# Layr-Labs/rust-kzg-bn254

Measured on AMD Instinct MI355X. Metric: G1-MSM (scalar,point) pairs/s = 2^20 x KZG coeff-form commitments/s, 2^20-point SRS, higher is better.
Workload: dtype int32x9 (29-bit limbs, 64-bit accumulate); 1 GPU; G1 MSM 2^20 scalars (KZG::commit_coeff_form), scalars resident in HBM; step k commits buffer k mod 8 (8 distinct resident scalar sets, 256 MiB); pipeline_depth=2, steps_per_launch=1

## Files before the change

rust-kzg-bn254_amd/csrc/curve_quad.h:

```cpp
#pragma once
#include "curve_pair.h"

#if defined(__HIPCC__)
namespace kzg {

struct QuadXyzz {
    Fq c;
    bool inf;
};

__device__ __forceinline__ void quad_set_inf(QuadXyzz& h) { fe_set_zero(h.c); h.inf = true; }

constexpr int QUAD_BCAST0 = 0x00, QUAD_BCAST1 = 0x55, QUAD_BCAST2 = 0xAA, QUAD_BCAST3 = 0xFF, QUAD_SWAP2 = 0x4E ;
template <int CTRL>
__device__ __forceinline__ int32_t quad_mov(int32_t x) {
#ifdef KZG_QUAD_NO_DPP
    const int lane = (int)(threadIdx.x & 63u);
    return __shfl(x, (lane & ~3) | ((CTRL >> (2 * (lane & 3))) & 3), 64);
#else
    return __builtin_amdgcn_mov_dpp(x, CTRL, 0xF, 0xF, true);
#endif
}
template <int CTRL>
__device__ __forceinline__ void fe_quad_mov(Fq& r, const Fq& a) {
// ... 93 lines not shown
    quad_add_tail(r, acc.c, df, sq, !acc.inf, from, q);
    if (acc.inf) r = from;
}

__device__ __forceinline__ void quad_dbl(QuadXyzz& r, const QuadXyzz& a, uint32_t q) {
    Fq y, u, s1, t1;
    fe_quad_mov<QUAD_BCAST1>(y, a.c);
    fe_dbl(u, y); fe_norm(u);
    fe_select(s1, q == 0u, a.c, u);
    fe_sqr(t1, s1);
    Fq m, m0, v1;
    fe_add(m, t1, t1); fe_add(m, m, t1); fe_norm(m);
    fe_quad_mov<QUAD_BCAST0>(m0, m);
    fe_quad_mov<QUAD_BCAST1>(v1, t1);
    Fq a2, b2, t2;
    fe_select(a2, q == 1u, u, a.c);
    fe_select(a2, q == 3u, m0, a2);
    fe_select(b2, q == 3u, m0, v1);
    fe_mul(t2, a2, b2);
    Fq mm, w1, x3, tq;
    fe_quad_mov<QUAD_BCAST3>(mm, t2);
    fe_quad_mov<QUAD_BCAST1>(w1, t2);
    fe_sub(x3, mm, t2); fe_sub(x3, x3, t2); fe_norm(x3);
    fe_add(tq, t2, t2); fe_add(tq, tq, t2); fe_sub(tq, tq, mm); fe_norm(tq);
    Fq a3, b3, t3;
    fe_select(a3, q == 0u, m, w1);
    fe_select(b3, q == 0u, tq, a.c);
    fe_mul(t3, a3, b3);
    Fq d0, y3;
    fe_quad_mov<QUAD_BCAST0>(d0, t3);
    fe_sub(y3, d0, t3); fe_norm(y3);
    Fq lo, hi;
    fe_select(lo, q == 1u, y3, x3);
    fe_select(hi, q == 3u, t3, t2);
    fe_select(r.c, q >= 2u, hi, lo);
    r.inf = false;
}
__device__ __forceinline__ void quad_dbl_any(QuadXyzz& r, const QuadXyzz& a, uint32_t q) {
    if (__all(a.inf)) { r = a; return; }
    QuadXyzz d;
    quad_dbl(d, a, q);
    if (a.inf) r = a; else r = d;
}

__device__ __forceinline__ void quad_load(QuadXyzz& h, const int32_t* __restrict__ base, size_t stride, size_t i, uint32_t q) {
#pragma unroll
    for (int j = 0; j < NL; ++j) h.c.l[j] = base[(size_t)(q * NL + j) * stride + i];
    const int z = fe_is_literal_zero(h.c) ? 1 : 0;
    h.inf = quad_mov<QUAD_BCAST2>(z) != 0;
}
__device__ __forceinline__ void quad_store(int32_t* __restrict__ base, size_t stride, size_t i, const QuadXyzz& h, uint32_t q) {
#pragma unroll
    for (int j = 0; j < NL; ++j) base[(size_t)(q * NL + j) * stride + i] = h.inf ? 0 : h.c.l[j];
}
__device__ __forceinline__ void quad_store_wire(uint32_t* __restrict__ out_wire, size_t i, const QuadXyzz& h, uint32_t q) {
    uint32_t w[8];
    if (h.inf) {
#pragma unroll
        for (int j = 0; j < 8; ++j) w[j] = 0;
    } else {
        fe_to_wire(w, h.c);
    }
    uint32_t* p = out_wire + i * 32 + q * 8;
    *reinterpret_cast<uint4*>(p) = make_uint4(w[0], w[1], w[2], w[3]);
    *reinterpret_cast<uint4*>(p + 4) = make_uint4(w[4], w[5], w[6], w[7]);
}
__device__ __forceinline__ void quad_shfl_down(QuadXyzz& r, const QuadXyzz& h, int d) {
#pragma unroll
    for (int j = 0; j < NL; ++j) r.c.l[j] = __shfl_down(h.c.l[j], d, 64);
    r.inf = __shfl_down((int)h.inf, d, 64) != 0;
}
__device__ __forceinline__ void quad_shfl(QuadXyzz& r, const QuadXyzz& h, int src) {
#pragma unroll
    for (int j = 0; j < NL; ++j) r.c.l[j] = __shfl(h.c.l[j], src, 64);
    r.inf = __shfl((int)h.inf, src, 64) != 0;
}

#ifndef KZG_PAIR_WAVES
#define KZG_PAIR_WAVES 3
#endif
#ifndef KZG_QUAD_SMALL_WAVES
#define KZG_QUAD_SMALL_WAVES 4
#endif
__device__ void group_zeta64(HalfXyzz& v, uint32_t lane, uint32_t w, bool odd, int32_t* __restrict__ lds);
__device__ void group_zeta64q(QuadXyzz& v, uint32_t lane, uint32_t w, uint32_t q, int32_t* __restrict__ lds);
struct PairLanes {
    using Point = HalfXyzz;
    using Role = bool;
    static constexpr uint32_t LANES = 2, GROUPS = 64 / LANES, LOG_GROUPS = 5;
    static constexpr int THREADS = 128, WAVES = KZG_PAIR_WAVES;
    static constexpr int ZETA_LDS_WORDS = 2 * NL * 64;
    static constexpr uint32_t FUSED_HEAVY = 12;
    static __device__ __forceinline__ Role role(uint32_t lane) { return (lane & 1u) != 0; }
    static __device__ __forceinline__ int affine_half(Role r) { return r ? 2 : 0; }
    static __device__ __forceinline__ void set_inf(Point& h) { half_set_inf(h); }
    static __device__ __forceinline__ void load(Point& h, const int32_t* __restrict__ base, size_t stride, size_t i, Role r) { half_load(h, base, stride, i, r); }
    static __device__ __forceinline__ void store(int32_t* __restrict__ base, size_t stride, size_t i, const Point& h, Role r) { half_store(base, stride, i, h, r); }
    static __device__ __forceinline__ void store_wire(uint32_t* __restrict__ out_wire, size_t i, const Point& h, Role r) { half_store_wire(out_wire, i, h, r); }
    static __device__ __forceinline__ void add(Point& r, const Point& a, const Point& b, Role role) { pair_add(r, a, b, role); }
    static __device__ __forceinline__ void madd(Point& r, const Point& acc, const Fq& c, uint32_t neg, Role role) { pair_madd(r, acc, c, neg, role); }
    static __device__ __forceinline__ void shfl_down(Point& r, const Point& h, int d) { half_shfl_down(r, h, d); }
    static __device__ __forceinline__ void shfl(Point& r, const Point& h, int src) { half_shfl(r, h, src); }
    static constexpr auto& zeta64 = group_zeta64;
};
struct QuadLanes {
    using Point = QuadXyzz;
    using Role = uint32_t;
    static constexpr uint32_t LANES = 4, GROUPS = 64 / LANES, LOG_GROUPS = 4;
    static constexpr int THREADS = 256, WAVES = KZG_QUAD_SMALL_WAVES;
    static constexpr int ZETA_LDS_WORDS = (NL + 1) * 256;
    static constexpr uint32_t FUSED_HEAVY = 8;
    static __device__ __forceinline__ Role role(uint32_t lane) { return lane & 3u; }
    static __device__ __forceinline__ int affine_half(Role r) { return (r & 1u) ? 2 : 0; }
    static __device__ __forceinline__ void set_inf(Point& h) { quad_set_inf(h); }
    static __device__ __forceinline__ void load(Point& h, const int32_t* __restrict__ base, size_t stride, size_t i, Role r) { quad_load(h, base, stride, i, r); }
    static __device__ __forceinline__ void store(int32_t* __restrict__ base, size_t stride, size_t i, const Point& h, Role r) { quad_store(base, stride, i, h, r); }
    static __device__ __forceinline__ void store_wire(uint32_t* __restrict__ out_wire, size_t i, const Point& h, Role r) { quad_store_wire(out_wire, i, h, r); }
    static __device__ __forceinline__ void add(Point& r, const Point& a, const Point& b, Role role) { quad_add(r, a, b, role); }
    static __device__ __forceinline__ void madd(Point& r, const Point& acc, const Fq& c, uint32_t neg, Role role) { quad_madd(r, acc, c, neg, role); }
    static __device__ __forceinline__ void shfl_down(Point& r, const Point& h, int d) { quad_shfl_down(r, h, d); }
    static __device__ __forceinline__ void shfl(Point& r, const Point& h, int src) { quad_shfl(r, h, src); }
    static constexpr auto& zeta64 = group_zeta64q;
};

}
#endif
```

rust-kzg-bn254_amd/csrc/msm.hip:

```cpp
#include "engine.h"
#include <new>
#include "msm_kernels.h"
#include "host_msm_epilogue.h"
#include "host_pairing.h"

#include <algorithm>
#include <cstdlib>
#include <chrono>
#include <cstdio>
#include <cstring>
#include <type_traits>
#include <vector>

namespace kzg {

void MsmWorkspace::release() {
    DeviceBuffer* all[] = {&scalars, &bases, &bases_wire, &digits, &sorted, &count, &blockbase, &sort_tmp, &sort_key, &sort_small, &offs, &block_sums,
                           &head, &cont, &blob, &bucket, &chunkS, &chunkTmp, &chunkA, &out_wire};
    for (auto* b : all) b->release();
    if (pinned_out) { (void)hipHostFree(pinned_out); pinned_out = nullptr; }
    if (ev_ready) { for (auto& e : ev) (void)hipEventDestroy(e); ev_ready = false; }
    if (ev_done) { (void)hipEventDestroy(ev_done); ev_done = nullptr; }
    if (ev_sorted) { (void)hipEventDestroy(ev_sorted); ev_sorted = nullptr; }
}
// ... 129 lines not shown
    hipStream_t st = L.st;
    const uint32_t n_total = p.n * p.batch;
    KZG_HIP_TRY(L.ctx, hipMemsetAsync(ws.count.p, 0, (size_t)p.G * 4, st));
    hipLaunchKernelGGL(k_msm_digits, dim3((n_total + 255) / 256), dim3(256), 0, st, L.d_scalars, n_total, p.n, p.c, p.W, ws.digits.as<uint32_t>(), (uint32_t*)nullptr);
    KZG_MARK(1);
    if (p.sort_small) {
        const uint32_t entries = (uint32_t)p.entries(), ge = (uint32_t)((p.entries() + 255) / 256);
        KZG_HIP_TRY(L.ctx, hipMemsetAsync(ws.blockbase.p, 0, (size_t)p.G * 4, st));
        hipLaunchKernelGGL(k_sort_small_hist, dim3(ge), dim3(256), 0, st, ws.digits.as<uint32_t>(), entries, p.set_len, p.B, ws.count.as<uint32_t>());
        scan_counts(L);
        KZG_MARK(2);
        hipLaunchKernelGGL(k_sort_small_scatter, dim3(ge), dim3(256), 0, st, ws.digits.as<uint32_t>(), entries, p.n, p.set_len, p.B,
                           ws.offs.as<uint32_t>(), ws.blockbase.as<uint32_t>(), p.idx_stride, (uint32_t)p.W, ws.sorted.as<uint32_t>());
    } else {
        const size_t lds_bytes = (size_t)p.B * 4;
        hipLaunchKernelGGL(k_sort_hist, dim3(p.tiles), dim3(256), lds_bytes, st, ws.digits.as<uint32_t>(), p.set_len, p.tile_len,
                           p.tiles_per_set, p.B, ws.count.as<uint32_t>(), ws.blockbase.as<uint32_t>());
        scan_counts(L);
        KZG_MARK(2);
        hipLaunchKernelGGL(k_sort_scatter, dim3(p.tiles), dim3(256), lds_bytes, st, ws.digits.as<uint32_t>(), p.n, p.set_len, p.tile_len,
                           p.tiles_per_set, p.B, ws.offs.as<uint32_t>(), ws.blockbase.as<uint32_t>(), p.idx_stride,
                           (uint32_t)p.W, ws.sorted.as<uint32_t>());
    }
    KZG_MARK(3);
    return KZG_OK;
}

static int32_t enqueue_sort(const Launch& L, const PolyPtrs* poly_ptrs) {
    const Plan& p = L.p;
    kzg_ctx* ctx = L.ctx;
    MsmWorkspace& ws = L.ws;
    if (p.bitsum) {
        for (int i = 0; i <= 4; ++i) KZG_MARK(i);
        return KZG_OK;
    }
    { int32_t rc = set_sort_lds_attributes(ctx); if (rc != KZG_OK) return rc; }
    const bool stagger = p.tables && p.polys >= 2;
    if (stagger && ctx->last_sorted && ctx->last_sorted_stream != L.st) KZG_HIP_TRY(ctx, hipStreamWaitEvent(L.st, ctx->last_sorted, 0));
    KZG_MARK(0);
    const uint32_t clean_g = ws.count_zero_ptr == ws.count.p ? ws.count_zero_g : 0;
    ws.count_zero_g = 0;
    const int32_t rc = p.sort2 ? sort_two_level(L, poly_ptrs) : p.lean_sort ? sort_lean(L, clean_g) : sort_from_digits(L);
    if (rc != KZG_OK) return rc;
    KZG_MARK(4);
    if (p.tables) {
        if (!ws.ev_sorted) KZG_HIP_TRY(ctx, hipEventCreateWithFlags(&ws.ev_sorted, hipEventDisableTiming));
        KZG_HIP_TRY(ctx, hipEventRecord(ws.ev_sorted, L.st));
        ctx->last_sorted = ws.ev_sorted;
        ctx->last_sorted_stream = L.st;
    }
    return KZG_OK;
}

static int32_t enqueue_accumulate(const Launch& L) {
    const Plan& p = L.p;
    MsmWorkspace& ws = L.ws;
    if (!p.bitsum && !p.fused)
        dispatch<true, false>(!L.bases.identity_free, [&](auto identity_bases) {
            hipLaunchKernelGGL(k_msm_accumulate<decltype(identity_bases)::value>, dim3(p.nl / 256), dim3(256), 0, L.st, L.bases.points, ws.sorted.as<uint32_t>(),
                               ws.offs.as<uint32_t>(), p.G, ws.head.as<int32_t>(), (size_t)p.G, ws.cont.as<int32_t>(), (size_t)p.nl, p.idx_log, p.stride_adj);
        });
    KZG_MARK(5);
    return KZG_OK;
}

static int32_t reduce_bitsum(const Launch& L) {
    const Plan& p = L.p;
    dispatch<8, 16, 32>(p.bitsum_chunk, [&](auto chunk) {
        hipLaunchKernelGGL(k_bitsum_level1<decltype(chunk)::value>, dim3(p.bitsum_wg), dim3(256), 0, L.st, L.bases.points, L.bases.table_stride, L.d_scalars, p.n,
                           L.ws.chunkS.as<int32_t>());
    });
    KZG_MARK(6);
    hipLaunchKernelGGL(k_bitsum_level2, dim3(p.n_out), dim3(256), 0, L.st, L.ws.chunkS.as<int32_t>(), p.bitsum_wg, L.d_out);
    return KZG_OK;
}

static int32_t reduce_tables(const Launch& L) {
    const Plan& p = L.p;
    MsmWorkspace& ws = L.ws;
    const uint32_t G1 = p.G1(), G1p = p.G1p();
    int32_t* x1 = ws.chunkS.as<int32_t>();
    dispatch<true, false>(p.quad1, [&](auto quads) {
        using LG = std::conditional_t<decltype(quads)::value, QuadLanes, PairLanes>;
        if (p.fused)
            hipLaunchKernelGGL(k_msm_bucket_bits1_fused<LG>, dim3(G1), dim3(LG::THREADS), 0, L.st, L.bases.points, ws.sorted.as<uint32_t>(), ws.offs.as<uint32_t>(), p.B,
                               p.idx_log, p.stride_adj, G1, x1, (size_t)7 * G1, L.d_out);
        else
            hipLaunchKernelGGL(k_msm_bucket_bits1<LG>, dim3(G1), dim3(LG::THREADS), 0, L.st, ws.offs.as<uint32_t>(), p.B, p.nl, ws.head.as<int32_t>(), (size_t)p.G,
                               ws.cont.as<int32_t>(), (size_t)p.nl, G1, x1, (size_t)7 * G1, L.d_out);
    });
    KZG_MARK(6);
    if (p.polys && p.c == 7) {
        hipLaunchKernelGGL(k_batch_finish, dim3((p.polys + 63) / 64), dim3(64), 0, L.st, x1, (size_t)7 * G1, G1, L.d_out);
    } else if (G1 > 1) {
        const uint32_t waves2 = 7 * G1p;
        if (p.quad)
            hipLaunchKernelGGL(k_red_bits2q, dim3(waves2), dim3(256), 0, L.st, x1, (size_t)7 * G1, G1, G1p, L.d_out);
        else
            hipLaunchKernelGGL(k_red_bits2p, dim3((waves2 + 1) / 2), dim3(128), 0, L.st, x1, (size_t)7 * G1, G1, G1p, L.d_out);
    }
    return KZG_OK;
}

static int32_t reduce_generic(const Launch& L) {
    const Plan& p = L.p;
    MsmWorkspace& ws = L.ws;
    hipStream_t st = L.st;
    const uint32_t n_chunks = p.n_chunks(), n_windows = p.n_windows();
    const uint32_t gg = (p.G + 255) / 256;
    hipLaunchKernelGGL(k_msm_bucket_fin, dim3(gg), dim3(256), 0, st, ws.offs.as<uint32_t>(), p.G, p.nl, p.m, n_chunks, ws.head.as<int32_t>(), (size_t)p.G,
                       ws.cont.as<int32_t>(), (size_t)p.nl, ws.bucket.as<int32_t>(), (size_t)p.G);
    const uint32_t gc = (n_chunks + 255) / 256;
    KZG_MARK(6);
    hipLaunchKernelGGL(k_red_chunk_sums, dim3(gc), dim3(256), 0, st, ws.bucket.as<int32_t>(), (size_t)p.G, n_chunks, p.m,
                       ws.chunkS.as<int32_t>(), (size_t)n_chunks);
    hipLaunchKernelGGL(k_red_suffix_scan, dim3(n_windows), dim3(p.T), 0, st, ws.chunkS.as<int32_t>(), ws.chunkTmp.as<int32_t>(),
                       (size_t)n_chunks, p.T);
    hipLaunchKernelGGL(k_red_chunk_running, dim3(gc), dim3(256), 0, st, ws.bucket.as<int32_t>(), (size_t)p.G,
                       ws.chunkS.as<int32_t>(), (size_t)n_chunks, n_chunks, p.T, p.m, ws.chunkA.as<int32_t>());
    hipLaunchKernelGGL(k_red_window_sum, dim3(n_windows), dim3(p.T), 0, st, ws.chunkA.as<int32_t>(), (size_t)n_chunks, p.T,
                       L.d_out);
    return KZG_OK;
}

static int32_t enqueue_reduce(const Launch& L) {
    const int32_t rc = L.p.bitsum ? reduce_bitsum(L) : L.p.tables ? reduce_tables(L) : reduce_generic(L);
    if (rc != KZG_OK) return rc;
    KZG_MARK(7);
    return KZG_OK;
}
#undef KZG_MARK

static PlanContext plan_context(const kzg_ctx* ctx) {
    PlanContext pc;
    pc.msm_c_override = ctx->msm_c_override;
    pc.msm_seg_override = ctx->msm_seg_override;
    pc.reduction_lanes = ctx->reduction_lanes;
    pc.acc_wave_slots = ctx->acc_wave_slots;
    for (int sl = 0; sl < KZG_NUM_SLOTS; ++sl) pc.other_in_flight |= ctx->slot_pending[sl] != nullptr;
    return pc;
}

static DeviceBuffer* ws_buffer(MsmWorkspace& ws, int which) {
    DeviceBuffer* const buffers[WS_BUFFERS] = {&ws.digits, &ws.sorted, &ws.count, &ws.sort_tmp, &ws.sort_key, &ws.sort_small, &ws.blockbase, &ws.offs, &ws.block_sums,
                                               &ws.head, &ws.cont, &ws.bucket, &ws.chunkS, &ws.chunkTmp, &ws.chunkA};
    return buffers[which];
}
int32_t msm_pinned_out(kzg_ctx* ctx, MsmWorkspace& ws) {
    if (ws.pinned_out) return KZG_OK;
    KZG_HIP_TRY(ctx, hipHostMalloc(&ws.pinned_out, (size_t)MSM_MAX_OUT * 32 * 4 + MSM_MAX_PARTS * 4, hipHostMallocDefault));
    KZG_HIP_TRY(ctx, hipHostGetDevicePointer(&ws.pinned_out_dev, ws.pinned_out, 0));
    return KZG_OK;
}
int32_t msm_sort_generic(kzg_ctx* ctx, MsmWorkspace& ws, hipStream_t st, const uint4* d_scalars, const Plan& p) {
    if (p.tables || p.batch != 1 || p.bitsum) return KZG_ERR_INVALID_ARG;
    for (int i : {WS_DIGITS, WS_SORTED, WS_COUNT, WS_BLOCKBASE, WS_OFFS, WS_BLOCK_SUMS}) KZG_HIP_TRY(ctx, ws_buffer(ws, i)->reserve(p.bytes[i]));
    const MsmBases none;
    const Launch L{ctx, ws, st, none, d_scalars, p, nullptr, false};
    const int32_t rc = enqueue_sort(L, nullptr);
    if (rc != KZG_OK) return rc;
    KZG_HIP_TRY(ctx, hipGetLastError());
    return KZG_OK;
}

static int32_t msm_enqueue(kzg_ctx* ctx, MsmWorkspace& ws, hipStream_t st, const MsmBases& bases, const uint4* d_scalars, size_t n,
                           uint32_t batch, Pending* pend, uint32_t out_off = 0, uint32_t out_cap = MSM_MAX_OUT, uint32_t polys = 0,
                           const PolyPtrs* poly_ptrs = nullptr) {
    const Plan p = make_plan(plan_context(ctx), n, bases, batch, polys);
    {
        const char* error = nullptr;
        const int32_t rc = msm_plan_status(p, bases, polys, out_off, out_cap, &error);
// ... 300 lines not shown
```

rust-kzg-bn254_amd/csrc/msm_kernels.h:

```cpp
#pragma once
#include <hip/hip_runtime.h>
#include "curve_pair.h"
#include "curve_quad.h"
#include "naf.h"
#include "msm_limits.h"

namespace kzg {

__device__ __forceinline__ void latency_bound_kernel() {
#if !defined(KZG_NO_SETPRIO)
    __builtin_amdgcn_s_setprio(3);
#endif
}

constexpr uint32_t DIGIT_NONE = 0xFFFFFFFFu;

__global__ void __launch_bounds__(256)
k_msm_digits(const uint4* __restrict__ scalars, uint32_t n_total, uint32_t n, int c, int W, uint32_t* __restrict__ digits,
             uint32_t* __restrict__ count = nullptr ) {
    latency_bound_kernel();
    uint32_t j = blockIdx.x * blockDim.x + threadIdx.x;
    if (j >= n_total) return;
    const uint32_t msm = j / n, i = j - msm * n;
    uint4 lo = scalars[2 * (size_t)j], hi = scalars[2 * (size_t)j + 1];
// ... 902 lines not shown
        xyzz_add(r, acc, v);
        acc = r;
    }
    xyzz_store(chunkS, chunk_stride, t, acc);
}
__global__ void __launch_bounds__(RED_T)
k_red_suffix_scan(int32_t* __restrict__ a, int32_t* __restrict__ b, size_t stride, uint32_t T) {
    uint32_t t = threadIdx.x;
    size_t base = (size_t)blockIdx.x * T;
    int32_t* src = a;
    int32_t* dst = b;
    for (uint32_t d = 1; d < T; d <<= 1) {
        if (t < T) {
            Xyzz v;
            xyzz_load(v, src, stride, base + t);
            if (t + d < T) {
                Xyzz u, r;
                xyzz_load(u, src, stride, base + t + d);
                xyzz_add(r, v, u);
                v = r;
            }
            xyzz_store(dst, stride, base + t, v);
        }
        __syncthreads();
        int32_t* tmp = src; src = dst; dst = tmp;
    }
    if (src != a && t < T) {
        Xyzz v;
        xyzz_load(v, src, stride, base + t);
        xyzz_store(a, stride, base + t, v);
    }
}
__global__ void __launch_bounds__(256)
k_red_chunk_running(const int32_t* __restrict__ bucket, size_t bucket_stride, const int32_t* __restrict__ suffix, size_t chunk_stride,
                    uint32_t n_chunks, uint32_t T, uint32_t m, int32_t* __restrict__ chunkA) {
    uint32_t t = blockIdx.x * blockDim.x + threadIdx.x;
    if (t >= n_chunks) return;
    Xyzz run, acc;
    if ((t % T) + 1 < T) xyzz_load(run, suffix, chunk_stride, t + 1);
    else xyzz_set_inf(run);
    xyzz_set_inf(acc);
    for (uint32_t k = m; k-- > 0;) {
        Xyzz v, r;
        xyzz_load(v, bucket, bucket_stride, (size_t)k * n_chunks + t);
        xyzz_add(r, run, v); run = r;
        xyzz_add(r, acc, run); acc = r;
    }
    xyzz_store(chunkA, chunk_stride, t, acc);
}
__global__ void __launch_bounds__(RED_T)
k_red_window_sum(int32_t* __restrict__ a, size_t stride, uint32_t T, uint32_t* __restrict__ out_wire) {
    uint32_t t = threadIdx.x;
    size_t base = (size_t)blockIdx.x * T;
    for (uint32_t d = T >> 1; d >= 1; d >>= 1) {
        if (t < d) {
            Xyzz v, u, r;
            xyzz_load(v, a, stride, base + t);
            xyzz_load(u, a, stride, base + t + d);
            xyzz_add(r, v, u);
            xyzz_store(a, stride, base + t, r);
        }
        __syncthreads();
    }
    if (t == 0) {
        Xyzz v;
        xyzz_load(v, a, stride, base);
        uint32_t w[32];
        xyzz_to_wire(w, v);
        for (int j = 0; j < 32; ++j) out_wire[(size_t)blockIdx.x * 32 + j] = w[j];
    }
}

__device__ __forceinline__ int zeta_role(uint32_t lane) {
    if (lane == 0) return 6;
    if ((lane & (lane - 1)) != 0) return -1;
    return __ffs((int)lane) - 1;
}
__device__ __forceinline__ void xyzz_store_wire(uint32_t* __restrict__ out_wire, size_t i, const Xyzz& v) {
    uint32_t w[32];
    xyzz_to_wire(w, v);
#pragma unroll
    for (int j = 0; j < 32; j += 4) *reinterpret_cast<uint4*>(out_wire + i * 32 + j) = make_uint4(w[j], w[j + 1], w[j + 2], w[j + 3]);
}
__device__ __forceinline__ void group_zeta64(HalfXyzz& v, uint32_t lane, uint32_t w, bool odd, int32_t* __restrict__ lds ) {
    const uint32_t pair = lane >> 1;
#pragma unroll 1
    for (int k = 0; k < 6; ++k) {
        HalfXyzz u;
        bool on;
        if (k < 5) {
            half_shfl_down(u, v, 2 << k);
            on = ((pair >> k) & 1u) == 0;
        } else {
            if (w == 1) {
#pragma unroll
                for (int j = 0; j < NL; ++j) { lds[j * 64 + lane] = v.inf ? 0 : v.u.l[j]; lds[(NL + j) * 64 + lane] = v.inf ? 0 : v.v.l[j]; }
            }
            __syncthreads();
#pragma unroll
            for (int j = 0; j < NL; ++j) { u.u.l[j] = lds[j * 64 + lane]; u.v.l[j] = lds[(NL + j) * 64 + lane]; }
            u.inf = fe_is_literal_zero(u.v);
            on = w == 0;
        }
        if (on) {
            HalfXyzz r;
            pair_add(r, v, u, odd);
            v = r;
        }
    }
}
__device__ __forceinline__ void group_zeta64q(QuadXyzz& v, uint32_t lane, uint32_t w, uint32_t q, int32_t* __restrict__ lds ) {
    const uint32_t quad = lane >> 2, tid = w * 64 + lane;
#pragma unroll 1
    for (int k = 0; k < 6; ++k) {
        QuadXyzz u;
        bool on;
        if (k < 4) {
            quad_shfl_down(u, v, 4 << k);
            on = ((quad >> k) & 1u) == 0;
        } else {
            const uint32_t bit = 1u << (k - 4);
            if (k == 5) __syncthreads();
            if (w & bit) {
#pragma unroll
                for (int j = 0; j < NL; ++j) lds[j * 256 + tid] = v.c.l[j];
                lds[NL * 256 + tid] = v.inf ? 1 : 0;
            }
            __syncthreads();
            on = (w & bit) == 0;
            const uint32_t src = tid + 64 * bit;
            if (on) {
#pragma unroll
                for (int j = 0; j < NL; ++j) u.c.l[j] = lds[j * 256 + src];
                u.inf = lds[NL * 256 + src] != 0;
            }
        }
        if (on) {
            QuadXyzz r;
            quad_add(r, v, u, q);
            v = r;
        }
    }
}

template <class LG>
__device__ __forceinline__ void bucket_partial_lanes(typename LG::Point& v, const BucketSpan& s, uint32_t k, const int32_t* __restrict__ head, size_t head_stride,
                                                     const int32_t* __restrict__ cont, size_t cont_stride, typename LG::Role role) {
    if (k == 0) { LG::load(v, head, head_stride, s.g, role); return; }
    LG::load(v, cont, cont_stride, bucket_cont_lane(s, k), role);
}
template <class LG>
__device__ __noinline__ void bucket_sum_heavy(typename LG::Point& tot, uint32_t g, uint32_t t1, uint32_t np, uint32_t long_run, uint32_t lane,
                                              const int32_t* __restrict__ head, size_t head_stride, const int32_t* __restrict__ cont, size_t cont_stride) {
    const uint32_t grp = lane / LG::LANES;
    const typename LG::Role role = LG::role(lane);
    BucketSpan h;
    h.g = g; h.t1 = t1; h.np = np; h.long_run = long_run != 0;
    typename LG::Point part;
    LG::set_inf(part);
    const uint32_t loads = (np + LG::GROUPS - 1) / LG::GROUPS;
#pragma unroll 1
    for (uint32_t step = 0; step < loads + LG::LOG_GROUPS; ++step) {
        typename LG::Point u;
        bool on;
        if (step < loads) {
            const uint32_t k = grp + LG::GROUPS * step;
            on = k < np;
            if (on) bucket_partial_lanes<LG>(u, h, k, head, head_stride, cont, cont_stride, role);
        } else {
            const uint32_t d = (LG::GROUPS / 2) >> (step - loads);
            LG::shfl_down(u, part, (int)(LG::LANES * d));
            on = grp < d;
        }
        if (on) {
            typename LG::Point r;
            LG::add(r, part, u, role);
            part = r;
        }
    }
    LG::shfl(tot, part, (int)(lane & (LG::LANES - 1)));
}
template <class LG>
__device__ __forceinline__ void bucket_sum_lanes(typename LG::Point& acc, const BucketSpan& s, uint32_t lane, typename LG::Role role, const int32_t* __restrict__ head,
                                                 size_t head_stride, const int32_t* __restrict__ cont, size_t cont_stride) {
    LG::set_inf(acc);
    const bool heavy = s.np > NP_SERIAL;
    if (!heavy) {
#pragma unroll 1
        for (uint32_t k = 0; k < s.np; ++k) {
            typename LG::Point v, r;
            bucket_partial_lanes<LG>(v, s, k, head, head_stride, cont, cont_stride, role);
            LG::add(r, acc, v, role);
            acc = r;
        }
    }
    unsigned long long todo = __ballot(heavy && (lane & (LG::LANES - 1)) == 0);
    while (todo) {
        const int src = __ffsll((long long)todo) - 1;
        todo &= todo - 1;
        typename LG::Point tot;
        bucket_sum_heavy<LG>(tot, __shfl(s.g, src, 64), __shfl(s.t1, src, 64), __shfl(s.np, src, 64), (uint32_t)__shfl((int)s.long_run, src, 64), lane,
                             head, head_stride, cont, cont_stride);
        if ((int)(lane & ~(LG::LANES - 1)) == src) acc = tot;
    }
}
template <class LG>
__global__ void __launch_bounds__(LG::THREADS) __attribute__((amdgpu_waves_per_eu(LG::WAVES, LG::WAVES)))
k_msm_bucket_bits1(const uint32_t* __restrict__ offs, uint32_t B, uint32_t nl, const int32_t* __restrict__ head, size_t head_stride,
                   const int32_t* __restrict__ cont, size_t cont_stride, uint32_t G1, int32_t* __restrict__ x1, size_t x_stride,
                   uint32_t* __restrict__ out_wire ) {
    latency_bound_kernel();
    __shared__ int32_t lds[LG::ZETA_LDS_WORDS];
    const uint32_t g = blockIdx.x, w = threadIdx.x >> 6, lane = threadIdx.x & 63, gp = w * LG::GROUPS + lane / LG::LANES;
    const typename LG::Role role = LG::role(lane);
    const uint32_t L = acc_seg_len(offs[B], nl);
    const uint32_t bkt = g * 64 + gp;
    BucketSpan s;
    s.g = bkt; s.t1 = 0; s.np = 0; s.long_run = false;
    if (bkt < B && L) s = bucket_span(offs, bkt, L);
    typename LG::Point v;
    bucket_sum_lanes<LG>(v, s, lane, role, head, head_stride, cont, cont_stride);
    LG::zeta64(v, lane, w, role, lds);
    const int zr = zeta_role(gp);
    if (zr < 0) return;
    if (G1 == 1) LG::store_wire(out_wire, (size_t)zr, v, role);
    else LG::store(x1, x_stride, (size_t)zr * G1 + g, v, role);
}
template <class LG>
__device__ __noinline__ void fused_heavy_bucket(typename LG::Point& tot, uint32_t hb, uint32_t he, uint32_t lane, const uint4* __restrict__ points,
                                                const uint32_t* __restrict__ sorted, uint32_t idx_log, uint32_t stride_adj) {
    const uint32_t grp = lane / LG::LANES;
    const typename LG::Role role = LG::role(lane);
    typename LG::Point part;
    LG::set_inf(part);
#pragma unroll 1
    for (uint32_t e = hb + grp; e < he; e += LG::GROUPS) {
        const uint32_t cur = sorted[e];
        const uint4* src = points + 4 * acc_point_index(cur & 0x7FFFFFFFu, idx_log, stride_adj) + LG::affine_half(role);
        const uint4 q0 = src[0], q1 = src[1];
        const uint32_t w32[8] = {q0.x, q0.y, q0.z, q0.w, q1.x, q1.y, q1.z, q1.w};
        int any = (q0.x | q0.y | q0.z | q0.w | q1.x | q1.y | q1.z | q1.w) != 0 ? 1 : 0;
        any |= pair_swap(any);
        if (!any) continue;
        Fq c;
        fe_unpack(c, w32);
        typename LG::Point r;
        LG::madd(r, part, c, cur >> 31, role);
        part = r;
    }
#pragma unroll 1
    for (int d = LG::GROUPS / 2; d >= 1; d >>= 1) {
        typename LG::Point u;
        LG::shfl_down(u, part, (int)LG::LANES * d);
        if (grp < (uint32_t)d) {
            typename LG::Point r;
            LG::add(r, part, u, role);
            part = r;
        }
    }
    LG::shfl(tot, part, (int)(lane & (LG::LANES - 1)));
}
template <class LG>
__global__ void __launch_bounds__(LG::THREADS) __attribute__((amdgpu_waves_per_eu(LG::WAVES, LG::WAVES)))
k_msm_bucket_bits1_fused(const uint4* __restrict__ points, const uint32_t* __restrict__ sorted, const uint32_t* __restrict__ offs, uint32_t B,
                         uint32_t idx_log, uint32_t stride_adj, uint32_t G1, int32_t* __restrict__ x1, size_t x_stride,
                         uint32_t* __restrict__ out_wire ) {
    latency_bound_kernel();
    __shared__ int32_t lds[LG::ZETA_LDS_WORDS];
    const uint32_t g = blockIdx.x, w = threadIdx.x >> 6, lane = threadIdx.x & 63, gp = w * LG::GROUPS + lane / LG::LANES;
    const typename LG::Role role = LG::role(lane);
    const uint32_t bkt = gp * G1 + g;
    uint32_t e = 0, end = 0;
    if (bkt < B) { e = offs[bkt]; end = offs[bkt + 1]; }
    const uint32_t hb = e, he = end;
    const bool heavy = end - e > LG::FUSED_HEAVY;
    if (heavy) end = e;
    typename LG::Point v;
    LG::set_inf(v);
    const uint32_t half = LG::affine_half(role);
    const uint32_t last = end ? end - 1 : 0;
    uint32_t ent = e < end ? sorted[e] : 0u;
    uint32_t ent1 = e < end ? sorted[e + 1 < end ? e + 1 : last] : 0u;
    const uint4* src = points + 4 * acc_point_index(ent & 0x7FFFFFFFu, idx_log, stride_adj) + half;
    uint4 q0 = make_uint4(0, 0, 0, 0), q1 = q0;
    if (e < end) { q0 = src[0]; q1 = src[1]; }
#pragma unroll 1
    for (; e < end; ++e) {
        const uint32_t cur = ent;
        const uint32_t w32[8] = {q0.x, q0.y, q0.z, q0.w, q1.x, q1.y, q1.z, q1.w};
        int any = (q0.x | q0.y | q0.z | q0.w | q1.x | q1.y | q1.z | q1.w) != 0 ? 1 : 0;
        ent = ent1;
        src = points + 4 * acc_point_index(ent & 0x7FFFFFFFu, idx_log, stride_adj) + half;
        q0 = src[0]; q1 = src[1];
        ent1 = sorted[e + 2 < end ? e + 2 : last];
        any |= pair_swap(any);
        if (!any) continue;
        Fq c;
        fe_unpack(c, w32);
        typename LG::Point r;
        LG::madd(r, v, c, cur >> 31, role);
        v = r;
    }
    unsigned long long todo = __ballot(heavy && (lane & (LG::LANES - 1)) == 0);
    while (todo) {
        const int src_lane = __ffsll((long long)todo) - 1;
        todo &= todo - 1;
        typename LG::Point tot;
        fused_heavy_bucket<LG>(tot, __shfl(hb, src_lane, 64), __shfl(he, src_lane, 64), lane, points, sorted, idx_log, stride_adj);
        if ((int)(lane & ~(LG::LANES - 1)) == src_lane) v = tot;
    }
    LG::zeta64(v, lane, w, role, lds);
    const int zr = zeta_role(gp);
    if (zr < 0) return;
    if (G1 == 1) LG::store_wire(out_wire, (size_t)zr, v, role);
    else LG::store(x1, x_stride, (size_t)zr * G1 + g, v, role);
}

__device__ __forceinline__ void group_zeta64_dual(HalfXyzz& vA, HalfXyzz& vB, uint32_t lane, uint32_t w, bool odd, int32_t* __restrict__ lds ) {
    const uint32_t gp = w * 32 + (lane >> 1);
#pragma unroll 1
    for (int k = 0; k < 6; ++k) {
        const bool bit = ((gp >> k) & 1u) != 0;
        HalfXyzz mine, pub, u, r;
        half_select(mine, bit, vB, vA);
        half_select(pub, bit, vA, vB);
        if (k < 5) {
            half_shfl_xor(u, pub, 2 << k);
        } else {
            int32_t* mine_slot = lds + w * (2 * NL * 64);
            const int32_t* other_slot = lds + (1 - w) * (2 * NL * 64);
#pragma unroll
            for (int j = 0; j < NL; ++j) { mine_slot[j * 64 + lane] = pub.inf ? 0 : pub.u.l[j]; mine_slot[(NL + j) * 64 + lane] = pub.inf ? 0 : pub.v.l[j]; }
            __syncthreads();
#pragma unroll
            for (int j = 0; j < NL; ++j) { u.u.l[j] = other_slot[j * 64 + lane]; u.v.l[j] = other_slot[(NL + j) * 64 + lane]; }
            u.inf = fe_is_literal_zero(u.v);
        }
        pair_add(r, mine, u, odd);
        half_select(vA, bit, vA, r);
        half_select(vB, bit, r, vB);
    }
}
__global__ void __launch_bounds__(128) __attribute__((amdgpu_waves_per_eu(KZG_PAIR_WAVES, KZG_PAIR_WAVES)))
k_red_bits2p(const int32_t* __restrict__ x1, size_t x_stride, uint32_t G1, uint32_t G1p, uint32_t* __restrict__ out_wire) {
    latency_bound_kernel();
    __shared__ int32_t lds[2 * 2 * NL * 64];
    const uint32_t w = threadIdx.x >> 6, lane = threadIdx.x & 63, gp = w * 32 + (lane >> 1);
    const bool odd = (lane & 1u) != 0;
    const uint32_t n_jobs = 7u * G1p;
    HalfXyzz v[2];
    bool sum_job[2];
    uint32_t job[2], grp[2];
#pragma unroll
    for (int which = 0; which < 2; ++which) {
        job[which] = 2 * blockIdx.x + which;
        const bool valid = job[which] < n_jobs;
        sum_job[which] = job[which] < 6u * G1p;
        const uint32_t a = sum_job[which] ? job[which] / G1p : 6u;
        grp[which] = sum_job[which] ? job[which] % G1p : job[which] - 6u * G1p;
        const uint32_t cnt = valid ? (G1 - grp[which] * 64 < 64 ? G1 - grp[which] * 64 : 64) : 0;
        const uint32_t idx = which ? 63 - gp : gp;
        if (idx < cnt) half_load(v[which], x1, x_stride, (size_t)a * G1 + (size_t)grp[which] * 64 + idx, odd);
        else half_set_inf(v[which]);
    }
    group_zeta64_dual(v[0], v[1], lane, w, odd, lds);
#pragma unroll
    for (int which = 0; which < 2; ++which) {
        if (job[which] >= n_jobs) continue;
        const uint32_t idx = which ? 63 - gp : gp;
        if (sum_job[which]) {
            if (idx == 0) half_store_wire(out_wire, job[which], v[which], odd);
        } else {
            const int role = zeta_role(idx);
            if (role >= 0) half_store_wire(out_wire, (size_t)6 * G1p + (size_t)role * G1p + grp[which], v[which], odd);
        }
    }
}
__global__ void __launch_bounds__(256) __attribute__((amdgpu_waves_per_eu(KZG_QUAD_SMALL_WAVES, KZG_QUAD_SMALL_WAVES)))
k_red_bits2q(const int32_t* __restrict__ x1, size_t x_stride, uint32_t G1, uint32_t G1p, uint32_t* __restrict__ out_wire) {
    latency_bound_kernel();
    __shared__ int32_t lds[(NL + 1) * 256];
    const uint32_t w = threadIdx.x >> 6, lane = threadIdx.x & 63, gp = w * 16 + (lane >> 2), q = lane & 3u;
    const uint32_t job = blockIdx.x;
    const bool sum_job = job < 6u * G1p;
    const uint32_t a = sum_job ? job / G1p : 6u;
    const uint32_t grp = sum_job ? job % G1p : job - 6u * G1p;
    const uint32_t cnt = G1 - grp * 64 < 64 ? G1 - grp * 64 : 64;
    QuadXyzz v;
    if (gp < cnt) quad_load(v, x1, x_stride, (size_t)a * G1 + (size_t)grp * 64 + gp, q);
    else quad_set_inf(v);
    group_zeta64q(v, lane, w, q, lds);
    if (sum_job) {
        if (gp == 0) quad_store_wire(out_wire, job, v, q);
    } else {
        const int role = zeta_role(gp);
        if (role >= 0) quad_store_wire(out_wire, (size_t)6 * G1p + (size_t)role * G1p + grp, v, q);
    }
}
// ... 134 lines not shown
```

Baseline: 965.4 million pairs/s.

## Replace pair-lane zeta64 reduction with LDS work-shared sum tree over two groups

For the pair-lane path, each workgroup now handles two bucket groups (256 threads), and the per-group 64-bucket subset-sum reduction is done as a shared-memory tree. At every level the add tasks are spread across all threads, instead of the old shuffle-down ladder where half the lanes sat idle at each step. The output stage is also reworked so threads write the seven zeta outputs from LDS. The aim is better lane utilisation in the reduction epilogue and fewer workgroups, at the cost of more LDS traffic, six block-wide barriers and a larger LDS footprint that may reduce occupancy.

New measurement: 977.1 million pairs/s, median of 6. 1.01x the previous value.

```diff
diff --git a/rust-kzg-bn254_amd/csrc/curve_quad.h b/rust-kzg-bn254_amd/csrc/curve_quad.h
--- a/rust-kzg-bn254_amd/csrc/curve_quad.h
+++ b/rust-kzg-bn254_amd/csrc/curve_quad.h
@@ -199,14 +199,13 @@
 #ifndef KZG_QUAD_SMALL_WAVES
 #define KZG_QUAD_SMALL_WAVES 4
 #endif
-__device__ void group_zeta64(HalfXyzz& v, uint32_t lane, uint32_t w, bool odd, int32_t* __restrict__ lds);
 __device__ void group_zeta64q(QuadXyzz& v, uint32_t lane, uint32_t w, uint32_t q, int32_t* __restrict__ lds);
 struct PairLanes {
     using Point = HalfXyzz;
     using Role = bool;
     static constexpr uint32_t LANES = 2, GROUPS = 64 / LANES, LOG_GROUPS = 5;
-    static constexpr int THREADS = 128, WAVES = KZG_PAIR_WAVES;
-    static constexpr int ZETA_LDS_WORDS = 2 * NL * 64;
+    static constexpr int TREE_GROUPS = 2, WG_GROUPS = TREE_GROUPS, THREADS = 128 * WG_GROUPS, WAVES = KZG_PAIR_WAVES;
+    static constexpr int SUMS_LDS_WORDS = 4 * NL * 64 * TREE_GROUPS;
     static constexpr uint32_t FUSED_HEAVY = 12;
     static __device__ __forceinline__ Role role(uint32_t lane) { return (lane & 1u) != 0; }
     static __device__ __forceinline__ int affine_half(Role r) { return r ? 2 : 0; }
@@ -218,14 +217,13 @@
     static __device__ __forceinline__ void madd(Point& r, const Point& acc, const Fq& c, uint32_t neg, Role role) { pair_madd(r, acc, c, neg, role); }
     static __device__ __forceinline__ void shfl_down(Point& r, const Point& h, int d) { half_shfl_down(r, h, d); }
     static __device__ __forceinline__ void shfl(Point& r, const Point& h, int src) { half_shfl(r, h, src); }
-    static constexpr auto& zeta64 = group_zeta64;
 };
 struct QuadLanes {
     using Point = QuadXyzz;
     using Role = uint32_t;
     static constexpr uint32_t LANES = 4, GROUPS = 64 / LANES, LOG_GROUPS = 4;
-    static constexpr int THREADS = 256, WAVES = KZG_QUAD_SMALL_WAVES;
-    static constexpr int ZETA_LDS_WORDS = (NL + 1) * 256;
+    static constexpr int TREE_GROUPS = 0, WG_GROUPS = 1, THREADS = 256 * WG_GROUPS, WAVES = KZG_QUAD_SMALL_WAVES;
+    static constexpr int SUMS_LDS_WORDS = (NL + 1) * 256;
     static constexpr uint32_t FUSED_HEAVY = 8;
     static __device__ __forceinline__ Role role(uint32_t lane) { return lane & 3u; }
     static __device__ __forceinline__ int affine_half(Role r) { return (r & 1u) ? 2 : 0; }
@@ -240,5 +238,31 @@
     static constexpr auto& zeta64 = group_zeta64q;
 };
 
-}
-#endif
+template <class LG, int NG>
+__device__ __forceinline__ void group_sum_tree(const typename LG::Point& v, uint32_t t, typename LG::Role role, int32_t* __restrict__ lds ) {
+    constexpr uint32_t SLOTS = 64 * NG;
+    LG::store(lds, SLOTS, t, v, role);
+    __syncthreads();
+#pragma unroll 1
+    for (uint32_t k = 0; k < 6; ++k) {
+        const uint32_t per_block = k + 1, per_group = per_block * (32u >> k), n_tasks = NG * per_group;
+        if ((t & ~(LG::GROUPS - 1)) < n_tasks) {
+            const bool on = t < n_tasks;
+            const uint32_t gr = t / per_group, rem = t - gr * per_group, blk = rem / per_block, j = rem - blk * per_block;
+            const uint32_t x = on ? gr * 64 + (blk << (k + 1)) + (j ? 1u << (j - 1) : 0u) : 0u;
+            typename LG::Point a, b, r;
+            LG::load(a, lds, SLOTS, x, role);
+            LG::load(b, lds, SLOTS, x + (1u << k), role);
+            if (!on) {
+                LG::set_inf(a);
+                LG::set_inf(b);
+            }
+            LG::add(r, a, b, role);
+            if (on) LG::store(lds, SLOTS, x, r, role);
+        }
+        __syncthreads();
+    }
+}
+
+}
+#endif
diff --git a/rust-kzg-bn254_amd/csrc/msm.hip b/rust-kzg-bn254_amd/csrc/msm.hip
--- a/rust-kzg-bn254_amd/csrc/msm.hip
+++ b/rust-kzg-bn254_amd/csrc/msm.hip
@@ -235,11 +235,12 @@
     int32_t* x1 = ws.chunkS.as<int32_t>();
     dispatch<true, false>(p.quad1, [&](auto quads) {
         using LG = std::conditional_t<decltype(quads)::value, QuadLanes, PairLanes>;
+        const uint32_t wgs = (G1 + LG::WG_GROUPS - 1) / LG::WG_GROUPS;
         if (p.fused)
-            hipLaunchKernelGGL(k_msm_bucket_bits1_fused<LG>, dim3(G1), dim3(LG::THREADS), 0, L.st, L.bases.points, ws.sorted.as<uint32_t>(), ws.offs.as<uint32_t>(), p.B,
+            hipLaunchKernelGGL(k_msm_bucket_bits1_fused<LG>, dim3(wgs), dim3(LG::THREADS), 0, L.st, L.bases.points, ws.sorted.as<uint32_t>(), ws.offs.as<uint32_t>(), p.B,
                                p.idx_log, p.stride_adj, G1, x1, (size_t)7 * G1, L.d_out);
         else
-            hipLaunchKernelGGL(k_msm_bucket_bits1<LG>, dim3(G1), dim3(LG::THREADS), 0, L.st, ws.offs.as<uint32_t>(), p.B, p.nl, ws.head.as<int32_t>(), (size_t)p.G,
+            hipLaunchKernelGGL(k_msm_bucket_bits1<LG>, dim3(wgs), dim3(LG::THREADS), 0, L.st, ws.offs.as<uint32_t>(), p.B, p.nl, ws.head.as<int32_t>(), (size_t)p.G,
                                ws.cont.as<int32_t>(), (size_t)p.nl, G1, x1, (size_t)7 * G1, L.d_out);
     });
     KZG_MARK(6);
diff --git a/rust-kzg-bn254_amd/csrc/msm_kernels.h b/rust-kzg-bn254_amd/csrc/msm_kernels.h
--- a/rust-kzg-bn254_amd/csrc/msm_kernels.h
+++ b/rust-kzg-bn254_amd/csrc/msm_kernels.h
@@ -1008,33 +1008,6 @@
 #pragma unroll
     for (int j = 0; j < 32; j += 4) *reinterpret_cast<uint4*>(out_wire + i * 32 + j) = make_uint4(w[j], w[j + 1], w[j + 2], w[j + 3]);
 }
-__device__ __forceinline__ void group_zeta64(HalfXyzz& v, uint32_t lane, uint32_t w, bool odd, int32_t* __restrict__ lds ) {
-    const uint32_t pair = lane >> 1;
-#pragma unroll 1
-    for (int k = 0; k < 6; ++k) {
-        HalfXyzz u;
-        bool on;
-        if (k < 5) {
-            half_shfl_down(u, v, 2 << k);
-            on = ((pair >> k) & 1u) == 0;
-        } else {
-            if (w == 1) {
-#pragma unroll
-                for (int j = 0; j < NL; ++j) { lds[j * 64 + lane] = v.inf ? 0 : v.u.l[j]; lds[(NL + j) * 64 + lane] = v.inf ? 0 : v.v.l[j]; }
-            }
-            __syncthreads();
-#pragma unroll
-            for (int j = 0; j < NL; ++j) { u.u.l[j] = lds[j * 64 + lane]; u.v.l[j] = lds[(NL + j) * 64 + lane]; }
-            u.inf = fe_is_literal_zero(u.v);
-            on = w == 0;
-        }
-        if (on) {
-            HalfXyzz r;
-            pair_add(r, v, u, odd);
-            v = r;
-        }
-    }
-}
 __device__ __forceinline__ void group_zeta64q(QuadXyzz& v, uint32_t lane, uint32_t w, uint32_t q, int32_t* __restrict__ lds ) {
     const uint32_t quad = lane >> 2, tid = w * 64 + lane;
 #pragma unroll 1
@@ -1066,6 +1039,30 @@
             quad_add(r, v, u, q);
             v = r;
         }
+    }
+}
+template <class LG, int NG>
+__device__ __forceinline__ void group_sum_tree_store(uint32_t t, typename LG::Role role, const int32_t* __restrict__ lds, uint32_t G1, int32_t* __restrict__ x1, size_t x_stride,
+                                                     uint32_t* __restrict__ out_wire) {
+    const uint32_t gr = t / 7, zr = t - gr * 7, g = blockIdx.x * NG + gr;
+    if (gr >= (uint32_t)NG || g >= G1) return;
+    typename LG::Point v;
+    LG::load(v, lds, 64 * NG, gr * 64 + (zr == 6 ? 0u : 1u << zr), role);
+    if (G1 == 1) LG::store_wire(out_wire, (size_t)zr, v, role);
+    else LG::store(x1, x_stride, (size_t)zr * G1 + g, v, role);
+}
+template <class LG>
+__device__ __forceinline__ void group_sums_out(typename LG::Point& v, uint32_t lane, uint32_t t, typename LG::Role role, int32_t* __restrict__ lds, uint32_t G1,
+                                               int32_t* __restrict__ x1, size_t x_stride, uint32_t* __restrict__ out_wire) {
+    if constexpr (LG::TREE_GROUPS != 0) {
+        group_sum_tree<LG, LG::TREE_GROUPS>(v, t, role, lds);
+        group_sum_tree_store<LG, LG::TREE_GROUPS>(t, role, lds, G1, x1, x_stride, out_wire);
+    } else {
+        LG::zeta64(v, lane, threadIdx.x >> 6, role, lds);
+        const int zr = zeta_role(t);
+        if (zr < 0) return;
+        if (G1 == 1) LG::store_wire(out_wire, (size_t)zr, v, role);
+        else LG::store(x1, x_stride, (size_t)zr * G1 + blockIdx.x, v, role);
     }
 }
 
@@ -1136,21 +1133,18 @@
                    const int32_t* __restrict__ cont, size_t cont_stride, uint32_t G1, int32_t* __restrict__ x1, size_t x_stride,
                    uint32_t* __restrict__ out_wire ) {
     latency_bound_kernel();
-    __shared__ int32_t lds[LG::ZETA_LDS_WORDS];
-    const uint32_t g = blockIdx.x, w = threadIdx.x >> 6, lane = threadIdx.x & 63, gp = w * LG::GROUPS + lane / LG::LANES;
+    constexpr int NG = LG::WG_GROUPS;
+    __shared__ int32_t lds[LG::SUMS_LDS_WORDS];
+    const uint32_t lane = threadIdx.x & 63, t = threadIdx.x / LG::LANES;
     const typename LG::Role role = LG::role(lane);
     const uint32_t L = acc_seg_len(offs[B], nl);
-    const uint32_t bkt = g * 64 + gp;
+    const uint32_t bkt = blockIdx.x * (64 * NG) + t;
     BucketSpan s;
     s.g = bkt; s.t1 = 0; s.np = 0; s.long_run = false;
     if (bkt < B && L) s = bucket_span(offs, bkt, L);
     typename LG::Point v;
     bucket_sum_lanes<LG>(v, s, lane, role, head, head_stride, cont, cont_stride);
-    LG::zeta64(v, lane, w, role, lds);
-    const int zr = zeta_role(gp);
-    if (zr < 0) return;
-    if (G1 == 1) LG::store_wire(out_wire, (size_t)zr, v, role);
-    else LG::store(x1, x_stride, (size_t)zr * G1 + g, v, role);
+    group_sums_out<LG>(v, lane, t, role, lds, G1, x1, x_stride, out_wire);
 }
 template <class LG>
 __device__ __noinline__ void fused_heavy_bucket(typename LG::Point& tot, uint32_t hb, uint32_t he, uint32_t lane, const uint4* __restrict__ points,
@@ -1192,12 +1186,14 @@
                          uint32_t idx_log, uint32_t stride_adj, uint32_t G1, int32_t* __restrict__ x1, size_t x_stride,
                          uint32_t* __restrict__ out_wire ) {
     latency_bound_kernel();
-    __shared__ int32_t lds[LG::ZETA_LDS_WORDS];
-    const uint32_t g = blockIdx.x, w = threadIdx.x >> 6, lane = threadIdx.x & 63, gp = w * LG::GROUPS + lane / LG::LANES;
+    constexpr int NG = LG::WG_GROUPS;
+    __shared__ int32_t lds[LG::SUMS_LDS_WORDS];
+    const uint32_t lane = threadIdx.x & 63, t = threadIdx.x / LG::LANES;
+    const uint32_t g = blockIdx.x * NG + t / 64, gp = t % 64;
     const typename LG::Role role = LG::role(lane);
     const uint32_t bkt = gp * G1 + g;
     uint32_t e = 0, end = 0;
-    if (bkt < B) { e = offs[bkt]; end = offs[bkt + 1]; }
+    if (g < G1 && bkt < B) { e = offs[bkt]; end = offs[bkt + 1]; }
     const uint32_t hb = e, he = end;
     const bool heavy = end - e > LG::FUSED_HEAVY;
     if (heavy) end = e;
@@ -1235,11 +1231,7 @@
         fused_heavy_bucket<LG>(tot, __shfl(hb, src_lane, 64), __shfl(he, src_lane, 64), lane, points, sorted, idx_log, stride_adj);
         if ((int)(lane & ~(LG::LANES - 1)) == src_lane) v = tot;
     }
-    LG::zeta64(v, lane, w, role, lds);
-    const int zr = zeta_role(gp);
-    if (zr < 0) return;
-    if (G1 == 1) LG::store_wire(out_wire, (size_t)zr, v, role);
-    else LG::store(x1, x_stride, (size_t)zr * G1 + g, v, role);
+    group_sums_out<LG>(v, lane, t, role, lds, G1, x1, x_stride, out_wire);
 }
 
 __device__ __forceinline__ void group_zeta64_dual(HalfXyzz& vA, HalfXyzz& vB, uint32_t lane, uint32_t w, bool odd, int32_t* __restrict__ lds ) {
```
